# KerkDovan/univer-ocr

Hardware: AMD Instinct MI355X
Metric: document-images/sec (fwd+bwd) on 256x512 synthetic pages (higher is better)
Workload: dtype f32; 1 GPU; BASELINE configs[2]: my_model train step (fwd+loss+bwd+L2+SGD) of Monochrome+Paragraph+Line on (32,256,512,1) pages and Char on (32,32,64,1) line strips per GPU; batch_per_gpu=32, global_batch=32, optimizer=sgd, parallelism=dp1, h2d_inclusive=False, input_grads=True, hip_graphs=True, pipelined_lanes=True, hw_queues=4

## Files before the change

univer-ocr_amd/csrc/conv_fast.hip:

```cpp
#include "finish_group.h"
#include "conv_dims.h"

namespace {

template <int C, typename TA>
__device__ __forceinline__ void load_vec(const TA* __restrict__ p, float (&v)[C]) {
    if constexpr (C == 1) {
        v[0] = ld1(p);
    } else if constexpr (C == 2) {
        const float2 t = ld2(p);
        v[0] = t.x;
        v[1] = t.y;
    } else {
        static_assert(C % 4 == 0, "channel count must be 1, 2 or a multiple of 4");
#pragma unroll
        for (int q = 0; q < C / 4; ++q) {
            const float4 t = ld4(p + 4 * q);
            v[4 * q] = t.x;
            v[4 * q + 1] = t.y;
            v[4 * q + 2] = t.z;
            v[4 * q + 3] = t.w;
        }
    }
}
// ... 696 lines not shown
};

template <int KH, int KW, int CIN, int COUT, int SH, int SW, int KYR, int COB, int PX, bool CLAMP, typename TA>
__global__ __launch_bounds__(256) void conv_wgrad_fast(const TA* __restrict__ x, const TA* __restrict__ dy,
                                                       float* __restrict__ partial, FastDims d, float pad,
                                                       int rows_per_block, int nbands) {
    using C = WgradCfg<KH, KW, CIN, COUT, SH, SW, KYR, COB>;
    constexpr int NXV = (PX - 1) * SW + KW;
    __shared__ float red[4][C::NP];
    const int lane = threadIdx.x, wv = threadIdx.y;
    const int band = blockIdx.x % nbands, b = blockIdx.x / nbands;
    const int kyg = blockIdx.y / C::OCG, ocg = blockIdx.y % C::OCG;
    const int ky0 = kyg * KYR, oc0 = ocg * COB;
    const int row0 = band * rows_per_block;
    const int row1 = min(d.oh, row0 + rows_per_block);
    float acc[C::NP];
#pragma unroll
    for (int a = 0; a < C::NP; ++a) acc[a] = 0.f;
    const TA* xb = x + (size_t)b * d.h * d.w * CIN;
    const TA* gb = dy + (size_t)b * d.oh * d.ow * COUT + oc0;
    for (int oy = row0 + wv; oy < row1; oy += 4) {
        for (int ox0 = lane * PX; ox0 < d.ow; ox0 += 64 * PX) {
            float g[PX][COB];
#pragma unroll
            for (int p = 0; p < PX; ++p) {
                if (ox0 + p < d.ow) {
                    load_vec<COB>(gb + ((size_t)oy * d.ow + ox0 + p) * COUT, g[p]);
                } else {
#pragma unroll
                    for (int o = 0; o < COB; ++o) g[p][o] = 0.f;
                }
                if (kyg == 0) {
#pragma unroll
                    for (int o = 0; o < COB; ++o) acc[C::NW + o] += g[p][o];
                }
            }
            const int iy0 = oy * SH - d.ph + ky0, ix0 = ox0 * SW - d.pw;
#pragma unroll
            for (int kyl = 0; kyl < KYR; ++kyl) {
                const int iy = iy0 + kyl;
                const bool row_ok = iy >= 0 && iy < d.h;
                const int iyc = min(max(iy, 0), d.h - 1);
                float xv[NXV][CIN];
                bool vec_done = false;
                if constexpr (CIN == 1 && PX % 4 == 0) {
                    constexpr int PWC = KW / 2, OFFS = (4 - PWC % 4) % 4;
                    if (d.pw == PWC && d.w % 4 == 0) {
                        load_row_c1<NXV, OFFS>(xb + (size_t)iyc * d.w, ix0 - OFFS, d.w, row_ok, pad, xv);
                        vec_done = true;
                    }
                }
                if (!vec_done) {
#pragma unroll
                    for (int j = 0; j < NXV; ++j) {
                        const int ix = ix0 + j;
                        if constexpr (CLAMP) {
                            load_vec<CIN>(xb + ((size_t)iyc * d.w + min(max(ix, 0), d.w - 1)) * CIN, xv[j]);
                            if (!(row_ok && ix >= 0 && ix < d.w)) {
#pragma unroll
                                for (int c = 0; c < CIN; ++c) xv[j][c] = pad;
                            }
                        } else {
                            if (row_ok && ix >= 0 && ix < d.w) {
                                load_vec<CIN>(xb + ((size_t)iy * d.w + ix) * CIN, xv[j]);
                            } else {
#pragma unroll
                                for (int c = 0; c < CIN; ++c) xv[j][c] = pad;
                            }
                        }
                    }
                }
#pragma unroll
                for (int kx = 0; kx < KW; ++kx)
#pragma unroll
                    for (int c = 0; c < CIN; ++c)
#pragma unroll
                        for (int o = 0; o < COB; ++o)
#pragma unroll
                            for (int p = 0; p < PX; ++p)
                                acc[((kyl * KW + kx) * CIN + c) * COB + o] += xv[p * SW + kx][c] * g[p][o];
            }
        }
    }
    lane_reduce_scatter<C::NP>(acc, lane);
    int base = 0;
#pragma unroll
    for (int s = 0; s < 6; ++s)
        if (lane & (32 >> s)) base += C::NP >> (s + 1);
#pragma unroll
    for (int r = 0; r < C::NP / 64; ++r) red[wv][base + r] = acc[r];
    __syncthreads();
    const int tid = wv * 64 + lane;
    float* out = partial + ((size_t)blockIdx.y * gridDim.x + blockIdx.x) * C::NP;
    for (int a = tid; a < C::NP; a += 256) out[a] = red[0][a] + red[1][a] + red[2][a] + red[3][a];
}

template <int KH, int KW, int CIN, int COUT, int KYR, int COB, int NW, int NP>
__global__ __launch_bounds__(256) void conv_wgrad_fast_finish(const float* __restrict__ partial, float* __restrict__ dw,
                                                              float* __restrict__ db, int nblocks, int use_bias,
                                                              int accumulate, float unscale) {
    __shared__ double smem[16];
    const int a = blockIdx.x, grp = blockIdx.y;
    constexpr int OCG = COUT / COB;
    const int kyg = grp / OCG, ocg = grp % OCG;
    const float* src = partial + (size_t)grp * nblocks * NP + a;
    double s = 0.0;
    for (int i = threadIdx.x; i < nblocks; i += blockDim.x) s += (double)src[(size_t)i * NP];
    s = block_reduce_sum(s, smem);
    if (threadIdx.x != 0) return;
    float* dst;
    if (a < NW) {
        const int o = a % COB, t = a / COB;
        const int c = t % CIN, tap = t / CIN;
        const int kx = tap % KW, kyl = tap / KW;
        dst = dw + (((size_t)(kyg * KYR + kyl) * KW + kx) * CIN + c) * COUT + ocg * COB + o;
    } else {
        if (kyg != 0) return;
        dst = db + ocg * COB + (a - NW);
        if (!use_bias) s = 0.0;
    }
    s *= (double)unscale;
    *dst = accumulate ? (float)((double)*dst + s) : (float)s;
}

namespace t542 {
constexpr int TH = 16, TW = 64, WH = TH + 4, WW = TW + 4, NW = 40, NB = 2, NACC = NW + NB, NP = 64;
__device__ __forceinline__ int swz(int row, int c) { return row * WW + (c & 3) * (WW / 4) + (c >> 2); }
struct Taprows {
    static constexpr int TH = t542::TH, TW = t542::TW, NW = t542::NW, NB = t542::NB, ROW = NACC;
};
}

template <typename TA>
__global__ __launch_bounds__(320) void conv_wgrad_t542(const TA* __restrict__ x, const TA* __restrict__ dy,
                                                       float* __restrict__ partial, int h, int wd, float pad,
                                                       int tiles_per_block) {
    using namespace t542;
    __shared__ float4 xs[WH * WW];
    __shared__ float2 gs[TH * TW];
    const int tid = threadIdx.x, lane = tid & 63, ky = tid >> 6;
    const int x0 = blockIdx.x * TW, b = blockIdx.z;
    const int tile0 = blockIdx.y * tiles_per_block, tiles_y = (h + TH - 1) / TH;
    const TA* xb = x + (size_t)b * h * wd * 4;
    const TA* gb = dy + (size_t)b * h * wd * 2;
    float acc[NP];
#pragma unroll
    for (int a = 0; a < NP; ++a) acc[a] = 0.f;
    const int cg = lane & 15, rsub = lane >> 4;
    const int t_end = min(tiles_y, tile0 + tiles_per_block);
    for (int t = tile0; t < t_end; ++t) {
        const int y0 = t * TH;
        __syncthreads();
        for (int e = tid; e < WH * WW; e += 320) {
            const int r = e / WW, c = e - r * WW;
            const int gy = y0 - 2 + r, gx = x0 - 2 + c;
            float4 v = ld4(xb + ((size_t)min(max(gy, 0), h - 1) * wd + min(max(gx, 0), wd - 1)) * 4);
            if (gy < 0 || gy >= h || gx < 0 || gx >= wd) v = make_float4(pad, pad, pad, pad);
            xs[swz(r, c)] = v;
        }
        for (int e = tid; e < TH * TW; e += 320) {
            const int r = e / TW, c = e - r * TW;
            const int gy = y0 + r, gx = x0 + c;
            float2 v = ld2(gb + ((size_t)min(gy, h - 1) * wd + min(gx, wd - 1)) * 2);
            if (gy >= h || gx >= wd) v = make_float2(0.f, 0.f);
            gs[e] = v;
        }
        __syncthreads();
#pragma unroll 1
        for (int it = 0; it < TH / 4; ++it) {
            const int r = it * 4 + rsub;
            float g[4][2];
            {
                const float4* gp = reinterpret_cast<const float4*>(gs + r * TW + 4 * cg);
                const float4 g01 = gp[0], g23 = gp[1];
                g[0][0] = g01.x, g[0][1] = g01.y, g[1][0] = g01.z, g[1][1] = g01.w;
                g[2][0] = g23.x, g[2][1] = g23.y, g[3][0] = g23.z, g[3][1] = g23.w;
            }
// ... 179 lines not shown
    {.kh = 5, .kw = 5, .cin = 4, .cout = 4, .sh = 2, .sw = 2,
     .fwd = {.px = 4}, .dx = {.py = 1}, .dw = {.kyr = 1, .cob = 4, .px = 2}},
    {.kh = 5, .kw = 5, .cin = 4, .cout = 4, .sh = 1, .sw = 1,
     .fwd = {.px = 4}, .dx = {.px = 4}, .dw = {.kyr = 1, .cob = 4, .px = 4}},
    {.kh = 5, .kw = 5, .cin = 4, .cout = 2, .sh = 1, .sw = 1,
     .fwd = {.px = 4}, .dx = {.px = 4}, .dw = {.kyr = 1, .cob = 2, .px = 4}},
    {.kh = 5, .kw = 3, .cin = 1, .cout = 64, .sh = 2, .sw = 1,
     .fwd = {.cob = 4, .py = 1}, .dx = {.py = 1}, .dw = {.kyr = 5, .cob = 8, .px = 1}},
};

template <int I>
struct FastConv {
    static constexpr FastRow R = FAST_CONVS[I];
    static constexpr int KH = R.kh, KW = R.kw, CIN = R.cin, COUT = R.cout, SH = R.sh, SW = R.sw;
    static_assert(R.fwd.px > 0 ? !R.fwd.cob && !R.fwd.py : R.fwd.cob > 0 && R.fwd.py > 0, "forward: px, or cob and py");
    static_assert(R.dx.px > 0 ? !R.dx.py && SH == 1 && SW == 1 : R.dx.py > 0, "dx: px (stride 1 only), or py");
    static_assert(R.dw.kyr > 0 && R.dw.cob > 0 && R.dw.px > 0, "dw: kyr, cob and px");
    static constexpr int FWD_KERNEL = R.fwd.px > 0 ? UOCR_CONV_TABLE_PX : UOCR_CONV_TABLE_FAST;
    static constexpr int DX_KERNEL = R.dx.px > 0 ? UOCR_CONV_TABLE_PX : UOCR_CONV_TABLE_FAST;

    static bool match(const ConvDims& d) {
        return d.kh == KH && d.kw == KW && d.cin == CIN && d.cout == COUT && d.sh == SH && d.sw == SW;
    }
    static FastDims dims(const ConvDims& d) { return FastDims{d.n, d.h, d.w, d.oh, d.ow, d.ph, d.pw}; }

    static int run(uocr_ctx* ctx, const ConvFwd& c) {
        const ConvDims& d = c.d;
        return uocr_act_tags<0>(ctx, c.act, UOCR_ACT_NONE, [&](auto kinds) -> int {
        using K = ActKindsIf<COUT == 4, decltype(kinds)>;
        UOCR_DISPATCH_TA(ctx, c.dtype, {
            if constexpr (R.fwd.px > 0) {
                const int groups = (d.ow + R.fwd.px - 1) / R.fwd.px;
                const dim3 grid((groups + 63) / 64, (d.oh + 3) / 4, d.n), block(64, 4);
                hipLaunchKernelGGL((conv_fwd_px<KH, KW, CIN, COUT, SH, SW, R.fwd.px, TA, K>), grid, block, 0, ctx->stream,
                                   (const TA*)c.x, (const float*)c.w, (const float*)c.b, (TA*)c.y, dims(d),
                                   (float)c.pad_value, c.use_bias, c.act, (float)c.act_alpha);
            } else {
                constexpr int PXW = 64 / (COUT / R.fwd.cob);
                const dim3 grid((d.ow + PXW - 1) / PXW, (d.oh + 4 * R.fwd.py - 1) / (4 * R.fwd.py), d.n), block(64, 4);
                hipLaunchKernelGGL((conv_fwd_fast<KH, KW, CIN, COUT, SH, SW, R.fwd.cob, R.fwd.py, TA>), grid, block, 0, ctx->stream,
                                   (const TA*)c.x, (const float*)c.w, (const float*)c.b, (TA*)c.y, dims(d),
                                   (float)c.pad_value, c.use_bias, c.act, (float)c.act_alpha);
            }
        });
        UOCR_LAUNCH_CHECK(ctx);
        return UOCR_OK;
        });
    }

    static int run(uocr_ctx* ctx, const ConvDgrad& c) {
        const ConvDims& d = c.d;
        UOCR_DISPATCH_TA(ctx, c.dtype, {
            if constexpr (R.dx.px > 0) {
                const int groups = (d.w + R.dx.px - 1) / R.dx.px;
                const dim3 grid((groups + 63) / 64, (d.h + 3) / 4, d.n), block(64, 4);
                hipLaunchKernelGGL((conv_dgrad_px<KH, KW, CIN, COUT, R.dx.px, TA>), grid, block, 0, ctx->stream,
                                   (const TA*)c.dy, (const float*)c.w, (TA*)c.dx, dims(d), (const TA*)c.mask.y,
                                   c.mask.act, (float)c.mask.alpha);
            } else {
                const dim3 grid((d.w + 63) / 64, (d.h + 4 * R.dx.py - 1) / (4 * R.dx.py), d.n), block(64, 4);
                hipLaunchKernelGGL((conv_dgrad_fast<KH, KW, CIN, COUT, SH, SW, R.dx.py, TA>), grid, block, 0, ctx->stream,
                                   (const TA*)c.dy, (const float*)c.w, (TA*)c.dx, dims(d), (const TA*)c.mask.y,
                                   c.mask.act, (float)c.mask.alpha);
            }
        });
        UOCR_LAUNCH_CHECK(ctx);
        return UOCR_OK;
    }

    static int run(uocr_ctx* ctx, const ConvWgrad& c) {
        const ConvDims& d = c.d;
        using C = WgradCfg<KH, KW, CIN, COUT, SH, SW, R.dw.kyr, R.dw.cob>;
        constexpr int RQ = 4;
        const int bands = ctx->opt_wgrad_bands > 0 ? ctx->opt_wgrad_bands : (C::NP >= 128 ? 64 : 512);
        int rows = (d.n * d.oh + bands - 1) / bands;
        rows = ((rows + RQ - 1) / RQ) * RQ;
        if (rows > d.oh) rows = ((d.oh + RQ - 1) / RQ) * RQ;
        const int nbands = (d.oh + rows - 1) / rows;
        const int nblocks = nbands * d.n, ngroups = C::KYG * C::OCG;
        const size_t bytes = (size_t)nblocks * ngroups * C::NP * sizeof(float);
        int rc = UOCR_OK;
        float* partial = uocr_partial_buffer(ctx, bytes, &rc);
        if (rc) return rc;
        UOCR_DISPATCH_TA(ctx, c.dtype, {
            hipLaunchKernelGGL((conv_wgrad_fast<KH, KW, CIN, COUT, SH, SW, R.dw.kyr, R.dw.cob, R.dw.px, (CIN >= 4), TA>),
                               dim3(nblocks, ngroups), dim3(64, 4), 0, ctx->stream, (const TA*)c.x, (const TA*)c.dy,
                               partial, dims(d), (float)c.pad_value, rows, nbands);
        });
        UOCR_LAUNCH_CHECK(ctx);
        const float unscale = (float)uocr_grad_unscale(c.dtype);
        const FinishDesc fd = finish_fast(partial, nblocks, ngroups, {C::NP, C::NW, KW, CIN, COUT, R.dw.kyr, R.dw.cob},
                                          (float*)c.dw, (float*)c.db, c.use_bias, c.accumulate, unscale);
        return uocr_finish(ctx, fd, [&] {
            hipLaunchKernelGGL((conv_wgrad_fast_finish<KH, KW, CIN, COUT, R.dw.kyr, R.dw.cob, C::NW, C::NP>),
                               dim3(C::NACC, ngroups), dim3(256), 0, ctx->stream, (const float*)partial, (float*)c.dw,
                               (float*)c.db, nblocks, c.use_bias, c.accumulate, unscale);
        });
    }
};

template <class F>
bool with_fast_conv(const ConvDims& d, F&& f) {
    return [&]<size_t... I>(std::index_sequence<I...>) {
        return ((FastConv<I>::match(d) && (f(FastConv<I>{}), true)) || ...);
    }(std::make_index_sequence<std::size(FAST_CONVS)>{});
}

struct C16Args { const void *src, *w, *bias; void* dst; float pad; int use_bias, act; float alpha; ActMask mask; };
template <class Kernel>
int launch_c16(uocr_ctx* ctx, Kernel kernel, int py, const C16Args& a, const ConvDims& d, int entry, int kernel_id) {
    const dim3 grid((d.w + 15) / 16, (d.h + 4 * py - 1) / (4 * py), d.n), block(64, 4);
    hipLaunchKernelGGL(kernel, grid, block, 0, ctx->stream, (const float*)a.src, (const float*)a.w, (const float*)a.bias,
                       (float*)a.dst, d.n, d.h, d.w, d.ph, d.pw, a.pad, a.use_bias, a.act, a.alpha,
                       (const float*)a.mask.y, a.mask.act, (float)a.mask.alpha);
    UOCR_LAUNCH_CHECK(ctx);
    uocr_note_conv(ctx, entry, kernel_id);
    return UOCR_OK;
}

bool fast_takes(uocr_ctx* ctx, int dtype, const ConvDims& d, const void* p0, const void* p1, const void* p2) {
    const int base = UOCR_DTYPE_BASE(dtype);
    if ((base != UOCR_F32 && base != UOCR_F16) || !ctx->opt_fast) return false;
    if (!uocr_aligned_act(p0, dtype) || !uocr_aligned_act(p1, dtype) || !uocr_aligned_act(p2, UOCR_F32)) return false;
    return with_fast_conv(d, [](auto) {});
}

}

bool uocr_conv_fast_takes(uocr_ctx* ctx, const ConvFwd& c) { return fast_takes(ctx, c.dtype, c.d, c.x, c.y, c.w); }
bool uocr_conv_fast_takes(uocr_ctx* ctx, const ConvDgrad& c) { return fast_takes(ctx, c.dtype, c.d, c.dy, c.dx, c.w); }
bool uocr_conv_fast_takes(uocr_ctx* ctx, const ConvWgrad& c) { return fast_takes(ctx, c.dtype, c.d, c.x, c.dy, c.dw); }

int uocr_conv_fast_run(uocr_ctx* ctx, const ConvFwd& c) {
    const ConvDims& d = c.d;
    const bool f32 = UOCR_DTYPE_BASE(c.dtype) == UOCR_F32;
    const C16Args c16{c.x, c.w, c.b, c.y, (float)c.pad_value, c.use_bias, c.act, (float)c.act_alpha, ActMask{nullptr, UOCR_ACT_NONE, 0.0}};
    if (f32 && is_c16_same(d, 1, 16))
        return launch_c16(ctx, conv_c16_expand<3, 3, 2, false>, 2, c16, d, 0, UOCR_CONV_C16_EXPAND);
    if (f32 && is_c16_same(d, 16, 1))
        return launch_c16(ctx, conv_c16_reduce<3, 3, 4, false>, 4, c16, d, 0, UOCR_CONV_C16_REDUCE);
    int rc = UOCR_OK;
    if (with_fast_conv(d, [&](auto fc) { rc = uocr_noted_conv(ctx, 0, fc.FWD_KERNEL, fc.run(ctx, c)); })) return rc;
    UOCR_FAIL(ctx, UOCR_ERR_UNSUPPORTED, "no fast conv kernel for this shape");
}

int uocr_conv_fast_run(uocr_ctx* ctx, const ConvDgrad& c) {
    const ConvDims& d = c.d;
    const bool f32 = UOCR_DTYPE_BASE(c.dtype) == UOCR_F32;
    const C16Args c16{c.dy, c.w, nullptr, c.dx, 0.f, 0, UOCR_ACT_NONE, 0.f, c.mask};
    if (f32 && is_c16_same(d, 16, 1))
        return launch_c16(ctx, conv_c16_expand<3, 3, 2, true>, 2, c16, d, 1, UOCR_CONV_C16_EXPAND);
    if (f32 && is_c16_same(d, 1, 16))
        return launch_c16(ctx, conv_c16_reduce<3, 3, 4, true>, 4, c16, d, 1, UOCR_CONV_C16_REDUCE);
    if (f32 && d.kh == 5 && d.kw == 3 && d.sh == 2 && d.sw == 1 && d.ph == 0 && d.pw == 1 && d.cin == 1 && d.cout == 64 &&
        d.h <= 65535 && d.n <= 65535) {
        hipLaunchKernelGGL(conv_dgrad_c64s2, dim3((unsigned)((d.w + 15) / 16), d.h, d.n), dim3(256), 0, ctx->stream,
                           (const float*)c.dy, (const float*)c.w, (float*)c.dx, d.n, d.h, d.w, d.oh, d.ow,
                           (const float*)c.mask.y, c.mask.act, (float)c.mask.alpha);
        UOCR_LAUNCH_CHECK(ctx);
        uocr_note_conv(ctx, 1, UOCR_CONV_DGRAD_C64S2);
        return UOCR_OK;
    }
    if (is_5x5_s2_pad2(d) && ((d.cin == 1 && (d.cout == 1 || d.cout == 4)) || (d.cin == 4 && d.cout == 4))) {
        const dim3 grid(((d.w + 1) / 2 + 63) / 64, ((d.h + 1) / 2 + 3) / 4, d.n), block(64, 4);
        const FastDims fd{d.n, d.h, d.w, d.oh, d.ow, d.ph, d.pw};
        const int rc = uocr_act_tags<1>(ctx, UOCR_ACT_NONE, c.mask.act, [&](auto kinds) -> int {
            using K = decltype(kinds);
            using D = ActKinds<UOCR_ACT_DYN, UOCR_ACT_DYN>;
            UOCR_DISPATCH_TA(ctx, c.dtype, {
                auto launch = [&](auto kernel) {
// ... 61 lines not shown
```

univer-ocr_amd/csrc/conv_up.hip:

```cpp
#include "up_phase.h"
#include "finish_group.h"
#include "conv_toeplitz.h"

namespace {

constexpr int CH = 4;
constexpr int RH = 16, RW = 32;
constexpr int XH = RH + 2, XW = RW + 2;
constexpr int XPLANE = 624;
constexpr int NWEFF = 9 * CH * 16;

__device__ __forceinline__ float weff_entry(const float* __restrict__ w, int i) {
    const int o = i & 3, phase = (i >> 2) & 3, c = (i >> 4) & 3, m = i >> 6;
    int ylo, yhi, xlo, xhi;
    tap_group(phase >> 1, m / 3, ylo, yhi);
    tap_group(phase & 1, m % 3, xlo, xhi);
    float v[2][2];
#pragma unroll
    for (int a = 0; a < 2; ++a)
#pragma unroll
        for (int b = 0; b < 2; ++b) v[a][b] = w[((min(ylo + a, 4) * 5 + min(xlo + b, 4)) * CH + c) * CH + o];
    float s = 0.f;
#pragma unroll
    for (int a = 0; a < 2; ++a)
// ... 225 lines not shown
constexpr int GH = 2 * (RH + 2), GW = 2 * (RW + 2);
template <typename TA, class K>
__global__ __launch_bounds__(256) void upconv_dgrad_kernel(const TA* __restrict__ dy, const float* __restrict__ weff,
                                                           TA* __restrict__ dxl, int hl, int wl,
                                                           const TA* __restrict__ mask_y, int mask_act,
                                                           float mask_alpha) {
    mask_act = act_kind<K::mask>(mask_act);
    __shared__ float4 gs[GH * GW];
    const int tid = threadIdx.x;
    const int rx = blockIdx.x * RW, ry = blockIdx.y * RH;
    const int H = 2 * hl, W = 2 * wl;
    const TA* gb = dy + (size_t)blockIdx.z * H * W * CH;
    if constexpr (sizeof(TA) == 4) {
        constexpr int NK = (GH * GW + 255) / 256;
        float4 v[NK];
        bool in[NK];
#pragma unroll
        for (int k = 0; k < NK; ++k) {
            const int i = min(tid + 256 * k, GH * GW - 1);
            const int r = i / GW, c = i - r * GW;
            const int gy = 2 * (ry - 1) + r, gx = 2 * (rx - 1) + c;
            in[k] = gy >= 0 && gy < H && gx >= 0 && gx < W;
            v[k] = ld4(gb + ((size_t)min(max(gy, 0), H - 1) * W + min(max(gx, 0), W - 1)) * CH);
        }
#pragma unroll
        for (int k = 0; k < NK; ++k)
            gs[min(tid + 256 * k, GH * GW - 1)] = in[k] ? v[k] : make_float4(0.f, 0.f, 0.f, 0.f);
    } else {
        for (int i = tid; i < GH * GW; i += 256) {
            const int r = i / GW, c = i - r * GW;
            const int gy = 2 * (ry - 1) + r, gx = 2 * (rx - 1) + c;
            float4 v = make_float4(0.f, 0.f, 0.f, 0.f);
            if (gy >= 0 && gy < H && gx >= 0 && gx < W) v = ld4(gb + ((size_t)gy * W + gx) * CH);
            gs[i] = v;
        }
    }
    const int c = tid & 31, r0 = tid >> 5;
    float4 yv[2];
    if (mask_act != UOCR_ACT_NONE) {
#pragma unroll
        for (int p = 0; p < 2; ++p)
            yv[p] = ld4(mask_y + (((size_t)blockIdx.z * hl + min(ry + r0 + 8 * p, hl - 1)) * wl + min(rx + c, wl - 1)) * CH);
    }
    __syncthreads();
    float acc[2][4];
#pragma unroll
    for (int p = 0; p < 2; ++p)
#pragma unroll
        for (int j = 0; j < 4; ++j) acc[p][j] = 0.f;
#pragma unroll 1
    for (int m = 0; m < 9; ++m) {
        const float* wt = weff + m * 64;
        const int my = m / 3 - 1, mx = m % 3 - 1;
#pragma unroll
        for (int p = 0; p < 2; ++p) {
            const int r = r0 + 8 * p;
            const float4* g0 = gs + (2 * (r - my + 1)) * GW + 2 * (c - mx + 1);
            const float4 g[4] = {g0[0], g0[1], g0[GW], g0[GW + 1]};
#pragma unroll
            for (int ch = 0; ch < 4; ++ch)
#pragma unroll
                for (int phase = 0; phase < 4; ++phase) {
                    const float* wv = wt + ch * 16 + phase * 4;
                    acc[p][ch] += wv[0] * g[phase].x + wv[1] * g[phase].y + wv[2] * g[phase].z + wv[3] * g[phase].w;
                }
        }
    }
#pragma unroll
    for (int p = 0; p < 2; ++p) {
        const int qy = ry + r0 + 8 * p, qx = rx + c;
        if (qy >= hl || qx >= wl) continue;
        const size_t off = (((size_t)blockIdx.z * hl + qy) * wl + qx) * CH;
        float4 out = make_float4(acc[p][0], acc[p][1], acc[p][2], acc[p][3]);
        if (mask_act != UOCR_ACT_NONE) {
            out.x *= act_grad_from_output<float>(yv[p].x, mask_act, mask_alpha);
            out.y *= act_grad_from_output<float>(yv[p].y, mask_act, mask_alpha);
            out.z *= act_grad_from_output<float>(yv[p].z, mask_act, mask_alpha);
            out.w *= act_grad_from_output<float>(yv[p].w, mask_act, mask_alpha);
        }
        st4(dxl + off, out);
    }
}

__device__ __forceinline__ void weff1_build(float (&we)[36], const float* __restrict__ w) {
#pragma unroll
    for (int m = 0; m < 9; ++m)
#pragma unroll
        for (int phase = 0; phase < 4; ++phase) {
            int ylo, yhi, xlo, xhi;
            tap_group(phase >> 1, m / 3, ylo, yhi);
            tap_group(phase & 1, m % 3, xlo, xhi);
            float s = 0.f;
            for (int ky = ylo; ky < yhi; ++ky)
                for (int kx = xlo; kx < xhi; ++kx) s += w[ky * 5 + kx];
            we[m * 4 + phase] = s;
        }
}

template <typename TA>
__global__ __launch_bounds__(256) void up1_fwd_kernel(const TA* __restrict__ xl, const float* __restrict__ w,
                                                      const float* __restrict__ bias, TA* __restrict__ y, int hl,
                                                      int wl, int use_bias, int act, float alpha) {
    __shared__ float xs[XH * XW];
    const int tid = threadIdx.x;
    const int rx = blockIdx.x * RW, ry = blockIdx.y * RH;
    const TA* xb = xl + (size_t)blockIdx.z * hl * wl;
    stage_batched<XH * XW, 256, 3, TA>(
        tid,
        [&](int i, bool& inside) {
            const int r = i / XW, c = i - r * XW;
            const int gy = ry - 1 + r, gx = rx - 1 + c;
            inside = gy >= 0 && gy < hl && gx >= 0 && gx < wl;
            return xb + (size_t)min(max(gy, 0), hl - 1) * wl + min(max(gx, 0), wl - 1);
        },
        [&](int i, TA v, bool inside) { xs[i] = inside ? (float)v : 0.f; });
    float we[36];
    weff1_build(we, w);
    const float b0 = use_bias ? bias[0] : 0.f;
    __syncthreads();
    const int c = tid & 31, r0 = tid >> 5;
    const int W = 2 * wl;
    TA* yb = y + (size_t)blockIdx.z * (2 * hl) * W;
#pragma unroll
    for (int p = 0; p < 2; ++p) {
        const int r = r0 + 8 * p, py = ry + r, pxl = rx + c;
        float acc[4] = {b0, b0, b0, b0};
#pragma unroll
        for (int m = 0; m < 9; ++m) {
            const float xv = xs[(r + m / 3) * XW + c + m % 3];
#pragma unroll
            for (int phase = 0; phase < 4; ++phase) acc[phase] += xv * we[m * 4 + phase];
        }
        if (py < hl && pxl < wl) {
            TA* o = yb + (size_t)(2 * py) * W + 2 * pxl;
            st2(o, make_float2(act_apply(acc[0], act, alpha), act_apply(acc[1], act, alpha)));
            st2(o + W, make_float2(act_apply(acc[2], act, alpha), act_apply(acc[3], act, alpha)));
        }
    }
}

template <typename TA>
__global__ __launch_bounds__(256) void up1_dgrad_kernel(const TA* __restrict__ dy, const float* __restrict__ w,
                                                        TA* __restrict__ dxl, int hl, int wl,
                                                        const TA* __restrict__ mask_y, int mask_act,
                                                        float mask_alpha) {
    __shared__ float gs[GH * GW];
    const int tid = threadIdx.x;
    const int rx = blockIdx.x * RW, ry = blockIdx.y * RH;
    const int H = 2 * hl, W = 2 * wl;
    const TA* gb = dy + (size_t)blockIdx.z * H * W;
    stage_batched<GH * GW, 256, 10, TA>(
        tid,
        [&](int i, bool& inside) {
            const int r = i / GW, c = i - r * GW;
            const int gy = 2 * (ry - 1) + r, gx = 2 * (rx - 1) + c;
            inside = gy >= 0 && gy < H && gx >= 0 && gx < W;
            return gb + (size_t)min(max(gy, 0), H - 1) * W + min(max(gx, 0), W - 1);
        },
        [&](int i, TA v, bool inside) { gs[i] = inside ? (float)v : 0.f; });
    float we[36];
    weff1_build(we, w);
    __syncthreads();
    const int c = tid & 31, r0 = tid >> 5;
#pragma unroll
    for (int p = 0; p < 2; ++p) {
        const int r = r0 + 8 * p;
        float acc = 0.f;
#pragma unroll
        for (int m = 0; m < 9; ++m) {
            const int my = m / 3 - 1, mx = m % 3 - 1;
            const float* g0 = gs + (2 * (r - my + 1)) * GW + 2 * (c - mx + 1);
            acc += we[m * 4] * g0[0] + we[m * 4 + 1] * g0[1] + we[m * 4 + 2] * g0[GW] + we[m * 4 + 3] * g0[GW + 1];
        }
        const int qy = ry + r, qx = rx + c;
        if (qy >= hl || qx >= wl) continue;
        const size_t off = ((size_t)blockIdx.z * hl + qy) * wl + qx;
        if (mask_act != UOCR_ACT_NONE) acc *= act_grad_from_output<float>(ld1(mask_y + off), mask_act, mask_alpha);
        st1(dxl + off, acc);
    }
}

template <typename TA>
__global__ __launch_bounds__(256) void up1_wgrad_kernel(const TA* __restrict__ xl, const TA* __restrict__ dy,
                                                        float* __restrict__ partial, int hl, int wl,
                                                        int rows_per_block) {
    __shared__ float xs[XH * XW];
    __shared__ float red[4][37];
    const int tid = threadIdx.x;
    const int rx = blockIdx.x * RW;
    const int row_begin = blockIdx.y * rows_per_block, row_end = min(hl, row_begin + rows_per_block);
    const TA* xb = xl + (size_t)blockIdx.z * hl * wl;
    const int W = 2 * wl;
    const TA* gb = dy + (size_t)blockIdx.z * (2 * hl) * W;
    const int c = tid & 31, r0 = tid >> 5;
    float acc[36], dbacc = 0.f;
#pragma unroll
    for (int i = 0; i < 36; ++i) acc[i] = 0.f;
    for (int ry = row_begin; ry < row_end; ry += RH) {
        __syncthreads();
        stage_batched<XH * XW, 256, 3, TA>(
            tid,
            [&](int i, bool& inside) {
                const int r = i / XW, cc = i - r * XW;
                const int gy = ry - 1 + r, gx = rx - 1 + cc;
                inside = gy >= 0 && gy < hl && gx >= 0 && gx < wl;
                return xb + (size_t)min(max(gy, 0), hl - 1) * wl + min(max(gx, 0), wl - 1);
            },
            [&](int i, TA v, bool inside) { xs[i] = inside ? (float)v : 0.f; });
        __syncthreads();
#pragma unroll
        for (int p = 0; p < 2; ++p) {
            const int r = r0 + 8 * p, py = ry + r, pxl = rx + c;
            if (py >= row_end || pxl >= wl) continue;
            const TA* g0 = gb + (size_t)(2 * py) * W + 2 * pxl;
            const float2 ga = ld2(g0), gbv = ld2(g0 + W);
            const float g[4] = {ga.x, ga.y, gbv.x, gbv.y};
            dbacc += (g[0] + g[1]) + (g[2] + g[3]);
#pragma unroll
            for (int m = 0; m < 9; ++m) {
                const float xv = xs[(r + m / 3) * XW + c + m % 3];
#pragma unroll
                for (int phase = 0; phase < 4; ++phase) acc[m * 4 + phase] += xv * g[phase];
            }
        }
    }
    const int lane = tid & 63, wv = tid >> 6;
#pragma unroll
    for (int i = 0; i < 36; ++i) {
        const float v = wave_reduce_sum(acc[i]);
        if (lane == 0) red[wv][i] = v;
    }
    dbacc = wave_reduce_sum(dbacc);
    if (lane == 0) red[wv][36] = dbacc;
    __syncthreads();
    const int blk = (blockIdx.z * gridDim.y + blockIdx.y) * gridDim.x + blockIdx.x;
    up1_write_row(partial + (size_t)blk * UP1_NOUT, [&](int i) { return red[0][i] + red[1][i] + red[2][i] + red[3][i]; }, tid);
}


int up_rows_per_block(int strips, int hl, int n, unsigned max_blocks = 2048u) {
    int rows = RH;
    while (rows < hl && (size_t)strips * ((hl + rows - 1) / rows) * n > max_blocks) rows += RH;
    return rows;
}

int check_up(uocr_ctx* ctx, int dtype, int n, int hl, int wl, int cin, int cout, int kh, int kw, int ph, int pw) {
    if (UOCR_DTYPE_BASE(dtype) != UOCR_F32 && UOCR_DTYPE_BASE(dtype) != UOCR_F16)
        UOCR_FAIL(ctx, UOCR_ERR_UNSUPPORTED, "upconv2x: float32 / float16 only");
    if (!((cin == CH && cout == CH) || (cin == 1 && cout == 1)) || kh != 5 || kw != 5 || ph != 2 || pw != 2)
        UOCR_FAIL(ctx, UOCR_ERR_UNSUPPORTED,
                  "upconv2x: 5x5 / padding 2 / 4 -> 4 or 1 -> 1 channels only (got %dx%d pad %d,%d %d -> %d)", kh, kw, ph,
                  pw, cin, cout);
    UOCR_REQUIRE(ctx, n > 0 && hl > 0 && wl > 0 && n <= 65535);
    return UOCR_OK;
}

ConvDims up_dims(int n, int hl, int wl, int cin, int cout) { return {n, hl, wl, cin, cout, 5, 5, 1, 1, 2, 2, 2 * hl, 2 * wl}; }
int up_ncols(const ConvWgrad& c) { return c.d.cin == 1 ? UP1_NOUT : UP4_NOUT; }

struct UpFwd { ConvFwd call; void* weff; };
struct UpDgrad { ConvDgrad call; const void* weff; };
template <class Up> bool up_h16_takes(uocr_ctx* ctx, const Up& u) { return uocr_upconv_h16_takes(ctx, u.call); }
template <class Up> int up_h16_run(uocr_ctx* ctx, const Up& u) { return uocr_upconv_h16_run(ctx, u.call); }
bool up_t32_takes(uocr_ctx* ctx, const UpDgrad& u) { return uocr_upconv_t32_takes(ctx, u.call); }
int up_t32_run(uocr_ctx* ctx, const UpDgrad& u) { return uocr_upconv_t32_run(ctx, u.call); }

int up_fwd_vector(uocr_ctx* ctx, const UpFwd& u) {
    const ConvFwd& c = u.call;
    const int n = c.d.n, hl = c.d.h, wl = c.d.w, cin = c.d.cin;
    const int strips = (wl + RW - 1) / RW, rows = up_rows_per_block(strips, hl, n, (unsigned)uocr_budget(ctx, 2048));
    if (cin != 1) uocr_note_split(ctx, (long long)strips * ((hl + rows - 1) / rows) * n, (long long)strips * ((hl + RH - 1) / RH) * n);
    return uocr_act_tags<0>(ctx, c.act, UOCR_ACT_NONE, [&](auto kinds) -> int {
    using K = decltype(kinds);
    UOCR_DISPATCH_TA(ctx, c.dtype, {
        if (cin == 1)
            hipLaunchKernelGGL((up1_fwd_kernel<TA>), dim3((wl + RW - 1) / RW, (hl + RH - 1) / RH, n), dim3(256), 0,
                               ctx->stream, (const TA*)c.x, (const float*)c.w, (const float*)c.b, (TA*)c.y, hl, wl,
                               c.use_bias, c.act, (float)c.act_alpha);
        else
            hipLaunchKernelGGL((upconv_fwd_kernel<TA, K>), dim3(strips, (hl + rows - 1) / rows, n), dim3(256), 0,
                               ctx->stream, (const TA*)c.x, (const float*)c.w, (const float*)c.b, (TA*)c.y, hl, wl, rows,
                               c.use_bias, c.act, (float)c.act_alpha, (float*)u.weff);
    });
    UOCR_LAUNCH_CHECK(ctx);
    return UOCR_OK;
    });
}

int up_dgrad_vector(uocr_ctx* ctx, const UpDgrad& u) {
    const ConvDgrad& c = u.call;
    const int n = c.d.n, hl = c.d.h, wl = c.d.w, cin = c.d.cin;
    const float* weff = (const float*)u.weff;
    if (cin != 1 && !weff) {
        const int rc = uocr_need_workspace(ctx, NWEFF * sizeof(float));
        if (rc != UOCR_OK) return rc;
        hipLaunchKernelGGL(upconv_weff_kernel, dim3(1), dim3(256), 0, ctx->stream, (const float*)c.w, (float*)ctx->workspace);
        weff = (const float*)ctx->workspace;
    }
    const dim3 grid((wl + RW - 1) / RW, (hl + RH - 1) / RH, n);
    return uocr_act_tags<1>(ctx, UOCR_ACT_NONE, c.mask.act, [&](auto kinds) -> int {
    using K = decltype(kinds);
    UOCR_DISPATCH_TA(ctx, c.dtype, {
        if (cin == 1)
            hipLaunchKernelGGL((up1_dgrad_kernel<TA>), grid, dim3(256), 0, ctx->stream, (const TA*)c.dy, (const float*)c.w,
                               (TA*)c.dx, hl, wl, (const TA*)c.mask.y, c.mask.act, (float)c.mask.alpha);
        else
            hipLaunchKernelGGL((upconv_dgrad_kernel<TA, K>), grid, dim3(256), 0, ctx->stream, (const TA*)c.dy,
                               weff, (TA*)c.dx, hl, wl, (const TA*)c.mask.y, c.mask.act, (float)c.mask.alpha);
    });
    UOCR_LAUNCH_CHECK(ctx);
    return UOCR_OK;
    });
}

int up_wgrad_finish(uocr_ctx* ctx, const ConvWgrad& c, const float* partial, int nblocks) {
    const float unscale = (float)uocr_grad_unscale(c.dtype);
// ... 82 lines not shown
```

univer-ocr_amd/csrc/uocr_common.h:

```cpp
#pragma once
#include <hip/hip_runtime.h>
#include <stdint.h>
#include <stdio.h>
#include <string.h>

#include <type_traits>
#include <utility>

#include "univer_hip.h"

enum uocr_report_id {
    UOCR_REPORT_SPLIT,
    UOCR_REPORT_GEMM,
    UOCR_REPORT_GEMM_GROUP,
    UOCR_REPORT_PAIR,
    UOCR_REPORT_CONV,
    UOCR_REPORT_LABEL,
    UOCR_REPORT_LABEL_BATCH,
    UOCR_REPORT_CHAR_LABEL,
    UOCR_REPORT_LINE_CROP,
    UOCR_REPORT_ROTATE,
    UOCR_REPORT_ROTATION_SEARCH,
    UOCR_REPORT_PRED_TO_TEXT,
    UOCR_REPORT_PACK_LINES,
// ... 114 lines not shown
        if (base_ == UOCR_F32) { using T = float; __VA_ARGS__; }                                  \
        else if (base_ == UOCR_F64) { using T = double; __VA_ARGS__; }                            \
        else if (base_ == UOCR_F16) { using T = _Float16; __VA_ARGS__; }                          \
        else UOCR_FAIL(ctx, UOCR_ERR_DTYPE, "unknown dtype %d", (int)(dtype));                    \
    } while (0)

static inline double uocr_grad_scale(int dtype) {
    return UOCR_DTYPE_BASE(dtype) == UOCR_F16 ? (double)(1u << (UOCR_DTYPE_GRAD_SCALE_LOG2(dtype) & 31)) : 1.0;
}
static inline double uocr_grad_unscale(int dtype) { return 1.0 / uocr_grad_scale(dtype); }

static inline int uocr_need_workspace(uocr_ctx* ctx, size_t bytes) {
    if (bytes > ctx->workspace_bytes)
        UOCR_FAIL(ctx, UOCR_ERR_WORKSPACE, "workspace too small: need %zu bytes, have %zu", bytes,
                  ctx->workspace_bytes);
    return UOCR_OK;
}

static inline unsigned uocr_blocks_for(size_t items, unsigned per_block, unsigned cap) {
    size_t b = (items + per_block - 1) / per_block;
    if (b < 1) b = 1;
    if (b > cap) b = cap;
    return (unsigned)b;
}

static inline long uocr_budget(const uocr_ctx* ctx, long budget) {
    return ctx->opt_max_blocks > 0 && ctx->opt_max_blocks < budget ? ctx->opt_max_blocks : budget;
}
static inline void uocr_note_split(uocr_ctx* ctx, long long blocks, long long items) {
    uocr_note(ctx, UOCR_REPORT_SPLIT, blocks, items);
}

template <typename K>
static inline int uocr_resident_blocks(uocr_ctx* ctx, K kernel, int threads, int* cache, int* out) {
    if (*cache == 0) {
        int nb = 0;
        UOCR_HIP(ctx, hipOccupancyMaxActiveBlocksPerMultiprocessor(&nb, kernel, threads, 0));
        *cache = nb > 0 ? nb : 1;
    }
    *out = *cache;
    return UOCR_OK;
}
template <typename K>
static inline int uocr_persistent_grid(uocr_ctx* ctx, K kernel, long ntiles, int slots_per_resident, int* cache,
                                       int* grid) {
    UOCR_REQUIRE(ctx, ntiles < (1l << 31));
    int resident = 0;
    const int rc = uocr_resident_blocks(ctx, kernel, 256, cache, &resident);
    if (rc != UOCR_OK) return rc;
    const long cap = uocr_budget(ctx, (long)ctx->cu_count * resident * slots_per_resident);
    *grid = (int)(ntiles < cap ? ntiles : cap);
    uocr_note_split(ctx, *grid, ntiles);
    return UOCR_OK;
}
static inline int uocr_tiles_per_block(int tiles_x, int tiles_y, int n, long budget) {
    int per_block = 1;
    while (per_block < tiles_y && (size_t)tiles_x * ((tiles_y + per_block - 1) / per_block) * n > (size_t)budget) ++per_block;
    return per_block;
}

static inline void uocr_note_pair(uocr_ctx* ctx, int kernel, int g, int mode, int pf, int nw, int blocks_x, int bands,
                                  int band_h) {
    uocr_note(ctx, UOCR_REPORT_PAIR, kernel, g, mode, pf, nw, blocks_x, bands, band_h);
}

static inline void uocr_note_conv(uocr_ctx* ctx, int entry, int kernel) {
    uocr_note(ctx, UOCR_REPORT_CONV, entry, kernel);
}
static inline int uocr_noted_conv(uocr_ctx* ctx, int entry, int kernel, int rc) {
    if (rc == UOCR_OK) uocr_note_conv(ctx, entry, kernel);
    return rc;
}

constexpr unsigned UOCR_MAX_GRID = 2048;
constexpr int UOCR_WAVE = 64;

template <typename T>
__device__ __forceinline__ T wave_reduce_sum(T v) {
#pragma unroll
    for (int off = 32; off > 0; off >>= 1) v += __shfl_down(v, off, 64);
    return v;
}

template <typename T>
__device__ __forceinline__ T wave_reduce_max(T v) {
#pragma unroll
    for (int off = 32; off > 0; off >>= 1) {
        T o = __shfl_down(v, off, 64);
        v = o > v ? o : v;
    }
    return v;
}

template <int NT = 0>
__device__ __forceinline__ double block_reduce_sum(double v, double* smem ) {
    const int lane = threadIdx.x & 63, wid = threadIdx.x >> 6;
    v = wave_reduce_sum(v);
    __syncthreads();
    if (lane == 0) smem[wid] = v;
    __syncthreads();
    const int nw = NT ? (NT + 63) >> 6 : (blockDim.x + 63) >> 6;
    v = (threadIdx.x < (unsigned)nw) ? smem[threadIdx.x] : 0.0;
    if (wid == 0) v = wave_reduce_sum(v);
    return v;
}

template <int NT = 0>
__device__ __forceinline__ double block_reduce_max(double v, double* smem ) {
    v = wave_reduce_max(v);
    __syncthreads();
    if ((threadIdx.x & 63) == 0) smem[threadIdx.x >> 6] = v;
    __syncthreads();
    if (threadIdx.x == 0) {
        const int nw = NT ? (NT + 63) >> 6 : (blockDim.x + 63) >> 6;
        for (int k = 1; k < nw; ++k) v = smem[k] > v ? smem[k] : v;
    }
    return v;
}

enum uocr_sync_word {
    UOCR_SYNC_SOFTMAX_CE = 1,
    UOCR_SYNC_SIGMOID_CE,
    UOCR_SYNC_OPT_TAIL,
    UOCR_SYNC_LABEL_STATS,
    UOCR_SYNC_WORDS
};
__device__ __forceinline__ void pub_store(double* p, double v) {
    __hip_atomic_store(p, v, __ATOMIC_RELAXED, __HIP_MEMORY_SCOPE_AGENT);
}
__device__ __forceinline__ double pub_load(const double* p) {
    return __hip_atomic_load(p, __ATOMIC_RELAXED, __HIP_MEMORY_SCOPE_AGENT);
}
__device__ __forceinline__ unsigned sync_arrive(unsigned* c) {
    asm volatile("s_waitcnt vmcnt(0)" ::: "memory");
    return __hip_atomic_fetch_add(c, 1u, __ATOMIC_RELAXED, __HIP_MEMORY_SCOPE_AGENT);
}
__device__ __forceinline__ void sync_clear(unsigned* c) {
    __hip_atomic_store(c, 0u, __ATOMIC_RELAXED, __HIP_MEMORY_SCOPE_AGENT);
}
struct FoldSum {
    static __device__ __forceinline__ double identity() { return 0.0; }
    static __device__ __forceinline__ double fold(double acc, double v) { return acc + v; }
    template <int B>
    static __device__ __forceinline__ double block(double v, double* smem) { return block_reduce_sum<B>(v, smem); }
};
struct FoldMax {
    static __device__ __forceinline__ double identity() { return -INFINITY; }
    static __device__ __forceinline__ double fold(double acc, double v) { return v > acc ? v : acc; }
    template <int B>
    static __device__ __forceinline__ double block(double v, double* smem) { return block_reduce_max<B>(v, smem); }
};
template <int B, int TRIPS, class... Op, size_t... S >
__device__ __forceinline__ bool last_block_fold_slots(std::index_sequence<S...>, unsigned* counter, double* partial,
                                                      double (&v)[sizeof...(Op)], double* smem) {
    constexpr int K = sizeof...(Op);
    static_assert(TRIPS >= 1 && K >= 1 && K * TRIPS <= 32, "a thread keeps K * TRIPS loads of two registers each in flight");
    if (threadIdx.x == 0) {
#pragma unroll
        for (int s = 0; s < K; ++s) pub_store(partial + (size_t)blockIdx.x * K + s, v[s]);
        smem[16] = sync_arrive(counter) == gridDim.x - 1 ? 1.0 : 0.0;
    }
    __syncthreads();
    if (smem[16] == 0.0) return false;
    const int count = (int)gridDim.x;
    double t[TRIPS][K];
#pragma unroll
// ... 160 lines not shown
```

Measured before the change: 34380 images/s.

## Add software-pipelined single-channel wgrad kernel and double-buffer up1 wgrad tiles

Adds a dedicated weight-gradient kernel for 1->1 channel convolutions that loads dy and x rows as whole 4-element vectors into two register buffers and alternates them, so loads for the next trip are in flight while the current one accumulates. The up1 wgrad kernel is restructured the same way: the next x tile and dy pairs are prefetched into registers while the current tile is summed, replacing the synchronous shared-memory staging. Both kernels, and the small-accumulator path of the generic wgrad, swap per-element wave reductions for a transpose-style shuffle reduction that finishes several sums in fewer shuffles. This costs more registers, which may lower occupancy, and adds clamped loads and edge masking that must match the old padding semantics.

```diff
diff --git a/univer-ocr_amd/csrc/conv_fast.hip b/univer-ocr_amd/csrc/conv_fast.hip
--- a/univer-ocr_amd/csrc/conv_fast.hip
+++ b/univer-ocr_amd/csrc/conv_fast.hip
@@ -802,17 +802,134 @@
             }
         }
     }
-    lane_reduce_scatter<C::NP>(acc, lane);
-    int base = 0;
-#pragma unroll
-    for (int s = 0; s < 6; ++s)
-        if (lane & (32 >> s)) base += C::NP >> (s + 1);
-#pragma unroll
-    for (int r = 0; r < C::NP / 64; ++r) red[wv][base + r] = acc[r];
+    if constexpr (C::NACC <= 32) {
+        float head[32];
+#pragma unroll
+        for (int a = 0; a < 32; ++a) head[a] = acc[a];
+        lane_transpose_reduce<32>(head, lane);
+        red[wv][(lane & 1) * 32 + (lane >> 1)] = (lane & 1) ? 0.f : head[0];
+    } else {
+        lane_reduce_scatter<C::NP>(acc, lane);
+        int base = 0;
+#pragma unroll
+        for (int s = 0; s < 6; ++s)
+            if (lane & (32 >> s)) base += C::NP >> (s + 1);
+#pragma unroll
+        for (int r = 0; r < C::NP / 64; ++r) red[wv][base + r] = acc[r];
+    }
     __syncthreads();
     const int tid = wv * 64 + lane;
     float* out = partial + ((size_t)blockIdx.y * gridDim.x + blockIdx.x) * C::NP;
     for (int a = tid; a < C::NP; a += 256) out[a] = red[0][a] + red[1][a] + red[2][a] + red[3][a];
+}
+
+template <typename TA>
+using Raw4 = std::conditional_t<std::is_same_v<TA, float>, float4, uocr_h4>;
+
+template <int KH, int KW, int SH, int SW, int PX, typename TA>
+__global__ __launch_bounds__(256) void conv_wgrad_c1(const TA* __restrict__ x, const TA* __restrict__ dy,
+                                                     float* __restrict__ partial, FastDims d, float pad,
+                                                     int rows_per_block, int nbands) {
+    using C = WgradCfg<KH, KW, 1, 1, SH, SW, KH, 1>;
+    using R4 = Raw4<TA>;
+    constexpr int NXV = (PX - 1) * SW + KW, PWC = KW / 2, OFFS = (4 - PWC % 4) % 4, NV4 = (OFFS + NXV + 3) / 4;
+    constexpr int NR = 32, NG4 = PX / 4;
+    static_assert(C::NACC <= NR && NR <= C::NP && PX % 4 == 0, "26 sums in rows of NP floats, whole 4-element loads of dy");
+    __shared__ float red[4][NR];
+    const int lane = threadIdx.x, wv = __builtin_amdgcn_readfirstlane(threadIdx.y);
+    const int band = blockIdx.x % nbands, b = blockIdx.x / nbands;
+    const int row0 = band * rows_per_block;
+    const int row1 = min(d.oh, row0 + rows_per_block);
+    const int trips = (d.ow + 64 * PX - 1) / (64 * PX);
+    float acc[NR];
+#pragma unroll
+    for (int a = 0; a < NR; ++a) acc[a] = 0.f;
+    const TA* xb = x + (size_t)b * d.h * d.w;
+    const TA* gb = dy + (size_t)b * d.oh * d.ow;
+    auto request = [&](R4 (&g)[NG4], R4 (&xv)[KH][NV4], int oy, int t) {
+        const int ox0 = (t * 64 + lane) * PX;
+#pragma unroll
+        for (int k = 0; k < NG4; ++k) g[k] = *reinterpret_cast<const R4*>(gb + (size_t)oy * d.ow + min(ox0 + 4 * k, d.ow - 4));
+        const int iy0 = oy * SH - d.ph, a4 = ox0 * SW - PWC - OFFS;
+#pragma unroll
+        for (int ky = 0; ky < KH; ++ky) {
+            const TA* row = xb + (size_t)min(max(iy0 + ky, 0), d.h - 1) * d.w;
+#pragma unroll
+            for (int k = 0; k < NV4; ++k) xv[ky][k] = *reinterpret_cast<const R4*>(row + min(max(a4 + 4 * k, 0), d.w - 4));
+        }
+    };
+    auto consume = [&](const R4 (&gr)[NG4], const R4 (&xr)[KH][NV4], int oy, int t) {
+        const int ox0 = (t * 64 + lane) * PX;
+        const bool live = ox0 < d.ow;
+        const float fill = live ? pad : 0.f;
+        float g[PX];
+#pragma unroll
+        for (int k = 0; k < NG4; ++k) {
+            const bool ok = ox0 + 4 * k < d.ow;
+            g[4 * k] = ok ? (float)gr[k].x : 0.f;
+            g[4 * k + 1] = ok ? (float)gr[k].y : 0.f;
+            g[4 * k + 2] = ok ? (float)gr[k].z : 0.f;
+            g[4 * k + 3] = ok ? (float)gr[k].w : 0.f;
+        }
+#pragma unroll
+        for (int p = 0; p < PX; ++p) acc[C::NW] += g[p];
+        const int iy0 = oy * SH - d.ph, a4 = ox0 * SW - PWC - OFFS;
+#pragma unroll
+        for (int ky = 0; ky < KH; ++ky) {
+            const bool row_ok = iy0 + ky >= 0 && iy0 + ky < d.h;
+            float buf[NV4 * 4];
+#pragma unroll
+            for (int k = 0; k < NV4; ++k) {
+                const int col = a4 + 4 * k;
+                const bool ok = live && row_ok && col >= 0 && col < d.w;
+                buf[4 * k] = ok ? (float)xr[ky][k].x : fill;
+                buf[4 * k + 1] = ok ? (float)xr[ky][k].y : fill;
+                buf[4 * k + 2] = ok ? (float)xr[ky][k].z : fill;
+                buf[4 * k + 3] = ok ? (float)xr[ky][k].w : fill;
+            }
+#pragma unroll
+            for (int kx = 0; kx < KW; ++kx)
+#pragma unroll
+                for (int p = 0; p < PX; ++p) acc[ky * KW + kx] += buf[OFFS + p * SW + kx] * g[p];
+        }
+    };
+    struct Trip {
+        int oy, t;
+    };
+    Trip ro{row0 + wv, 0}, co = ro, last = ro;
+    auto next = [&](Trip& s) {
+        const Trip was = s;
+        if (++s.t == trips) s.t = 0, s.oy += 4;
+        return was;
+    };
+    auto next_request = [&] {
+        if (ro.oy < row1) last = next(ro);
+        return last;
+    };
+    auto consume_next = [&](const R4 (&gr)[NG4], const R4 (&xr)[KH][NV4]) {
+        const Trip c = next(co);
+        consume(gr, xr, c.oy, c.t);
+    };
+    const int n = row0 + wv < row1 ? ((row1 - row0 - wv + 3) / 4) * trips : 0;
+    R4 ga[NG4], gz[NG4], xa[KH][NV4], xz[KH][NV4];
+    for (int pass = 0; 2 * pass < n; ++pass) {
+        if (pass > 0) consume_next(ga, xa);
+        const Trip ra = next_request();
+        request(ga, xa, ra.oy, ra.t);
+        __builtin_amdgcn_sched_barrier(0);
+        if (pass > 0) consume_next(gz, xz);
+        const Trip rz = next_request();
+        request(gz, xz, rz.oy, rz.t);
+        __builtin_amdgcn_sched_barrier(0);
+    }
+    if (n > 0) consume_next(ga, xa);
+    if (n > 0 && co.oy < row1) consume_next(gz, xz);
+    lane_transpose_reduce<NR>(acc, lane);
+    if ((lane & 1) == 0) red[wv][lane >> 1] = acc[0];
+    __syncthreads();
+    const int tid = wv * 64 + lane;
+    float* out = partial + (size_t)blockIdx.x * C::NP;
+    if (tid < C::NP) out[tid] = tid < NR ? red[0][tid] + red[1][tid] + red[2][tid] + red[3][tid] : 0.f;
 }
 
 template <int KH, int KW, int CIN, int COUT, int KYR, int COB, int NW, int NP>
@@ -1158,10 +1275,21 @@
         int rc = UOCR_OK;
         float* partial = uocr_partial_buffer(ctx, bytes, &rc);
         if (rc) return rc;
+        constexpr bool C1 = CIN == 1 && COUT == 1 && C::KYG == 1 && R.dw.px % 4 == 0;
         UOCR_DISPATCH_TA(ctx, c.dtype, {
-            hipLaunchKernelGGL((conv_wgrad_fast<KH, KW, CIN, COUT, SH, SW, R.dw.kyr, R.dw.cob, R.dw.px, (CIN >= 4), TA>),
-                               dim3(nblocks, ngroups), dim3(64, 4), 0, ctx->stream, (const TA*)c.x, (const TA*)c.dy,
-                               partial, dims(d), (float)c.pad_value, rows, nbands);
+            bool done = false;
+            if constexpr (C1) {
+                if (d.pw == KW / 2 && d.w % 4 == 0 && d.ow % 4 == 0) {
+                    hipLaunchKernelGGL((conv_wgrad_c1<KH, KW, SH, SW, R.dw.px, TA>), dim3(nblocks), dim3(64, 4), 0,
+                                       ctx->stream, (const TA*)c.x, (const TA*)c.dy, partial, dims(d), (float)c.pad_value,
+                                       rows, nbands);
+                    done = true;
+                }
+            }
+            if (!done)
+                hipLaunchKernelGGL((conv_wgrad_fast<KH, KW, CIN, COUT, SH, SW, R.dw.kyr, R.dw.cob, R.dw.px, (CIN >= 4), TA>),
+                                   dim3(nblocks, ngroups), dim3(64, 4), 0, ctx->stream, (const TA*)c.x, (const TA*)c.dy,
+                                   partial, dims(d), (float)c.pad_value, rows, nbands);
         });
         UOCR_LAUNCH_CHECK(ctx);
         const float unscale = (float)uocr_grad_unscale(c.dtype);
diff --git a/univer-ocr_amd/csrc/conv_up.hip b/univer-ocr_amd/csrc/conv_up.hip
--- a/univer-ocr_amd/csrc/conv_up.hip
+++ b/univer-ocr_amd/csrc/conv_up.hip
@@ -331,6 +331,8 @@
     }
 }
 
+template <typename TA>
+using Up1Pair = std::conditional_t<std::is_same_v<TA, float>, float2, uocr_h2>;
 __device__ __forceinline__ void weff1_build(float (&we)[36], const float* __restrict__ w) {
 #pragma unroll
     for (int m = 0; m < 9; ++m)
@@ -433,8 +435,9 @@
 __global__ __launch_bounds__(256) void up1_wgrad_kernel(const TA* __restrict__ xl, const TA* __restrict__ dy,
                                                         float* __restrict__ partial, int hl, int wl,
                                                         int rows_per_block) {
-    __shared__ float xs[XH * XW];
-    __shared__ float red[4][37];
+    using G2 = Up1Pair<TA>;
+    __shared__ float xs[XH * XW + 1];
+    __shared__ float red[4][40];
     const int tid = threadIdx.x;
     const int rx = blockIdx.x * RW;
     const int row_begin = blockIdx.y * rows_per_block, row_end = min(hl, row_begin + rows_per_block);
@@ -442,28 +445,42 @@
     const int W = 2 * wl;
     const TA* gb = dy + (size_t)blockIdx.z * (2 * hl) * W;
     const int c = tid & 31, r0 = tid >> 5;
+    int xr[3], xg[3];
+#pragma unroll
+    for (int k = 0; k < 3; ++k) {
+        const int i = min(tid + 256 * k, XH * XW - 1);
+        xr[k] = i / XW - 1;
+        xg[k] = rx - 1 + i % XW;
+    }
+    const int gcol = 2 * min(rx + c, wl - 1);
+    auto load_tile = [&](TA (&xv)[3], G2 (&g)[2][2], int ry) {
+#pragma unroll
+        for (int k = 0; k < 3; ++k)
+            xv[k] = xb[(size_t)min(max(ry + xr[k], 0), hl - 1) * wl + min(max(xg[k], 0), wl - 1)];
+        __builtin_amdgcn_sched_barrier(0);
+#pragma unroll
+        for (int p = 0; p < 2; ++p) {
+            const TA* g0 = gb + (size_t)(2 * min(ry + r0 + 8 * p, hl - 1)) * W + gcol;
+            g[p][0] = *reinterpret_cast<const G2*>(g0);
+            g[p][1] = *reinterpret_cast<const G2*>(g0 + W);
+        }
+    };
+    auto put_tile = [&](const TA (&xv)[3], int ry) {
+#pragma unroll
+        for (int k = 0; k < 3; ++k) {
+            const int gy = ry + xr[k];
+            xs[min(tid + 256 * k, XH * XW)] = gy >= 0 && gy < hl && xg[k] >= 0 && xg[k] < wl ? (float)xv[k] : 0.f;
+        }
+    };
     float acc[36], dbacc = 0.f;
 #pragma unroll
     for (int i = 0; i < 36; ++i) acc[i] = 0.f;
-    for (int ry = row_begin; ry < row_end; ry += RH) {
-        __syncthreads();
-        stage_batched<XH * XW, 256, 3, TA>(
-            tid,
-            [&](int i, bool& inside) {
-                const int r = i / XW, cc = i - r * XW;
-                const int gy = ry - 1 + r, gx = rx - 1 + cc;
-                inside = gy >= 0 && gy < hl && gx >= 0 && gx < wl;
-                return xb + (size_t)min(max(gy, 0), hl - 1) * wl + min(max(gx, 0), wl - 1);
-            },
-            [&](int i, TA v, bool inside) { xs[i] = inside ? (float)v : 0.f; });
-        __syncthreads();
+    auto sum_tile = [&](const G2 (&gv)[2][2], int ry) {
 #pragma unroll
         for (int p = 0; p < 2; ++p) {
             const int r = r0 + 8 * p, py = ry + r, pxl = rx + c;
             if (py >= row_end || pxl >= wl) continue;
-            const TA* g0 = gb + (size_t)(2 * py) * W + 2 * pxl;
-            const float2 ga = ld2(g0), gbv = ld2(g0 + W);
-            const float g[4] = {ga.x, ga.y, gbv.x, gbv.y};
+            const float g[4] = {(float)gv[p][0].x, (float)gv[p][0].y, (float)gv[p][1].x, (float)gv[p][1].y};
             dbacc += (g[0] + g[1]) + (g[2] + g[3]);
 #pragma unroll
             for (int m = 0; m < 9; ++m) {
@@ -472,15 +489,33 @@
                 for (int phase = 0; phase < 4; ++phase) acc[m * 4 + phase] += xv * g[phase];
             }
         }
+    };
+    TA xa[3], xz[3];
+    G2 ga[2][2], gz[2][2];
+    load_tile(xa, ga, row_begin);
+    for (int ry = row_begin; ry < row_end; ry += 2 * RH) {
+        __syncthreads();
+        put_tile(xa, ry);
+        __syncthreads();
+        load_tile(xz, gz, ry + RH < row_end ? ry + RH : ry);
+        __builtin_amdgcn_sched_barrier(0);
+        sum_tile(ga, ry);
+        if (ry + RH >= row_end) break;
+        __syncthreads();
+        put_tile(xz, ry + RH);
+        __syncthreads();
+        load_tile(xa, ga, ry + 2 * RH < row_end ? ry + 2 * RH : ry + RH);
+        __builtin_amdgcn_sched_barrier(0);
+        sum_tile(gz, ry + RH);
     }
     const int lane = tid & 63, wv = tid >> 6;
-#pragma unroll
-    for (int i = 0; i < 36; ++i) {
-        const float v = wave_reduce_sum(acc[i]);
-        if (lane == 0) red[wv][i] = v;
-    }
-    dbacc = wave_reduce_sum(dbacc);
-    if (lane == 0) red[wv][36] = dbacc;
+    float head[32], tail[8] = {acc[32], acc[33], acc[34], acc[35], dbacc, 0.f, 0.f, 0.f};
+#pragma unroll
+    for (int i = 0; i < 32; ++i) head[i] = acc[i];
+    lane_transpose_reduce<32>(head, lane);
+    lane_transpose_reduce<8>(tail, lane);
+    if ((lane & 1) == 0) red[wv][lane >> 1] = head[0];
+    if ((lane & 7) == 0) red[wv][32 + (lane >> 3)] = tail[0];
     __syncthreads();
     const int blk = (blockIdx.z * gridDim.y + blockIdx.y) * gridDim.x + blockIdx.x;
     up1_write_row(partial + (size_t)blk * UP1_NOUT, [&](int i) { return red[0][i] + red[1][i] + red[2][i] + red[3][i]; }, tid);
diff --git a/univer-ocr_amd/csrc/uocr_common.h b/univer-ocr_amd/csrc/uocr_common.h
--- a/univer-ocr_amd/csrc/uocr_common.h
+++ b/univer-ocr_amd/csrc/uocr_common.h
@@ -220,6 +220,33 @@
     return v;
 }
 
+template <int NP, int S>
+__device__ __forceinline__ void lane_transpose_reduce_step(float (&acc)[NP], int lane) {
+    constexpr int bit = 32 >> S;
+    if constexpr ((NP >> S) > 1) {
+        constexpr int half = NP >> (S + 1);
+        const bool up = lane & bit;
+#pragma unroll
+        for (int i = 0; i < half; ++i) {
+            const float send = up ? acc[i] : acc[i + half];
+            const float keep = up ? acc[i + half] : acc[i];
+            acc[i] = keep + __shfl_xor(send, bit, 64);
+        }
+    } else {
+        acc[0] += __shfl_xor(acc[0], bit, 64);
+    }
+}
+template <int NP>
+__device__ __forceinline__ void lane_transpose_reduce(float (&acc)[NP], int lane) {
+    static_assert(NP >= 1 && NP <= 64 && (NP & (NP - 1)) == 0, "a power of two up to the wave size");
+    lane_transpose_reduce_step<NP, 0>(acc, lane);
+    lane_transpose_reduce_step<NP, 1>(acc, lane);
+    lane_transpose_reduce_step<NP, 2>(acc, lane);
+    lane_transpose_reduce_step<NP, 3>(acc, lane);
+    lane_transpose_reduce_step<NP, 4>(acc, lane);
+    lane_transpose_reduce_step<NP, 5>(acc, lane);
+}
+
 template <typename T>
 __device__ __forceinline__ T wave_reduce_max(T v) {
 #pragma unroll
```

Measured after the change: 34540 images/s, median of 6. Within noise of the previous version (+0.5%).
